# mfalxa/fakepta

Measured on AMD Instinct MI355X. Metric: residual samples/sec (TOA×realization) for 100-psr HD GWB; % FP64 peak, higher is better.
Workload: dtype f64

## Files before the change

fakepta_amd/_capi.py:

```python
import ctypes
import os
import threading

import numpy as np

_HERE = os.path.dirname(os.path.abspath(__file__))
_DEFAULT_LIB = os.path.join(_HERE, "lib", "libfakepta_amd.so")
LIB_PATH = os.environ.get("FAKEPTA_AMD_LIB", _DEFAULT_LIB)

if not os.path.exists(LIB_PATH):
    raise ImportError(
        f"fakepta_amd: HIP library not found at {LIB_PATH}. Build it with "
        "`python -c 'import __graft_entry__ as g; g.build()'` (or `make -C fakepta_amd/csrc`).")

_lib = ctypes.CDLL(LIB_PATH)

_c_int = ctypes.c_int
_i32, _i64, _u64 = ctypes.c_int32, ctypes.c_int64, ctypes.c_uint64
_dbl = ctypes.c_double
_vp = ctypes.c_void_p
_ctx_p = ctypes.c_void_p

_SIGS = [
    ("fpta_version", _c_int, []),
# ... 24 lines not shown
    ("fpta_batch_download", _c_int, [_ctx_p, _i32, _i32, _vp]),
    ("fpta_batch_device_out", _c_int, [_ctx_p, ctypes.POINTER(_vp), ctypes.POINTER(_i64), ctypes.POINTER(_i32)]),
    ("fpta_batch_checksums", _c_int, [_ctx_p, _vp]),
    ("fpta_batch_synth_checksums", _c_int, [_ctx_p, _u64, _i64, _i64, _i32, _vp]),
    ("fpta_batch_correlations", _c_int, [_ctx_p, _i32, _vp]),
    ("fpta_batch_info", _c_int, [_ctx_p, _vp]),
    ("fpta_batch_grid_info", _c_int, [_ctx_p, _vp]),
    ("fpta_batch_grid_info_n", _c_int, [_ctx_p, _vp, _i32]),
    ("fpta_set_option", _c_int, [_ctx_p, _i32, _i64]),
    ("fpta_kernel_stats", _c_int, [_ctx_p, _i32, ctypes.POINTER(_i64), ctypes.POINTER(_dbl)]),
    ("fpta_reset_stats", _c_int, [_ctx_p]),
    ("fpta_synchronize", _c_int, [_ctx_p]),
    ("fpta_debug_philox", _c_int, [_ctx_p, _i64, _vp, _vp, _vp]),
    ("fpta_debug_normals", _c_int, [_ctx_p, _i64, _vp, _vp]),
    ("fpta_debug_fill_out", _c_int, [_ctx_p, _dbl]),
    ("fpta_get_option", _c_int, [_ctx_p, _i32, ctypes.POINTER(_i64)]),
    ("fpta_build_flags", _c_int, []),
    ("fpta_batch_path_reason", ctypes.c_char_p, [_ctx_p]),
    ("fpta_multi_create", _c_int, [_i32, _vp, ctypes.POINTER(_vp)]),
    ("fpta_multi_destroy", _c_int, [_vp]),
    ("fpta_multi_last_error", ctypes.c_char_p, [_vp]),
    ("fpta_multi_size", _c_int, [_vp]),
    ("fpta_multi_context", _ctx_p, [_vp, _i32]),
    ("fpta_multi_set_toas", _c_int, [_vp, _i32, _vp, _vp, _vp]),
    ("fpta_multi_add_signal", _c_int, [_vp, _i32, _i32, _vp, _vp, _dbl, _dbl, _vp, _vp]),
    ("fpta_multi_set_white", _c_int, [_vp, _vp, _i64, _vp, _vp, _vp]),
    ("fpta_multi_set_option", _c_int, [_vp, _i32, _i64]),
    ("fpta_multi_synth", _c_int, [_vp, _u64, _i64, _i64, _i32, _vp]),
    ("fpta_multi_set_gather", _c_int, [_vp, _i32]),
    ("fpta_multi_last_gather", _c_int, [_vp]),
    ("fpta_comm_unique_id", _c_int, [_vp]),
    ("fpta_comm_init_rank", _c_int, [_ctx_p, _i32, _i32, _vp, ctypes.POINTER(_vp)]),
    ("fpta_comm_destroy", _c_int, [_vp]),
    ("fpta_comm_last_error", ctypes.c_char_p, [_vp]),
    ("fpta_comm_size", _c_int, [_vp, ctypes.POINTER(_i32), ctypes.POINTER(_i32)]),
    ("fpta_comm_max", _c_int, [_vp, ctypes.POINTER(_dbl)]),
    ("fpta_comm_gather", _c_int, [_vp, _vp, _i64, _vp]),
]
_OPTIONAL = {"fpta_debug_normals"}
for _name, _res, _args in _SIGS:
    try:
        _fn = getattr(_lib, _name)
    except AttributeError:
        if _name in _OPTIONAL and LIB_PATH != _DEFAULT_LIB:
            continue
        raise
    _fn.restype = _res
    _fn.argtypes = _args

EXPORTED = [s[0] for s in _SIGS]

OPT_SYNTH_PATH, OPT_MFMA_MIN_REAL, OPT_PROFILE, OPT_ANCHOR, OPT_VALU_VARIANT, OPT_FUSE_WHITE = 1, 2, 3, 4, 5, 6
OPT_GRID_WIDTH, OPT_GRID_SIGMA, OPT_GRID_MFMA, OPT_FUSE_CHECKSUMS = 7, 8, 9, 10
OPT_MIX_MFMA, OPT_OVERLAP, OPT_INTERP_LDS, OPT_GRID_COALESCE, OPT_INTERP_WS, OPT_SIDE_SPLIT = 11, 12, 13, 14, 15, 16
# ... 359 lines not shown
    def kernel_stats(self, which):
        n, ms = _i64(), _dbl()
        self._check(_lib.fpta_kernel_stats(self._h, int(which), ctypes.byref(n), ctypes.byref(ms)),
                    "fpta_kernel_stats")
        return n.value, ms.value

    def reset_stats(self):
        self._check(_lib.fpta_reset_stats(self._h), "fpta_reset_stats")

    def synchronize(self):
        self._check(_lib.fpta_synchronize(self._h), "fpta_synchronize")

    def debug_fill_out(self, value):
        self._check(_lib.fpta_debug_fill_out(self._h, float(value)), "fpta_debug_fill_out")

    def debug_philox(self, ctr, key):
        ctr = np.ascontiguousarray(ctr, dtype=np.uint32).reshape(-1, 4)
        key = np.ascontiguousarray(key, dtype=np.uint32)
        out = np.empty_like(ctr)
        self._check(_lib.fpta_debug_philox(self._h, len(ctr), _ptr(ctr), _ptr(key), _ptr(out)), "fpta_debug_philox")
        return out

    def debug_normals(self, words):
        words = np.ascontiguousarray(words, dtype=np.uint32).reshape(-1, 4)
        out = np.empty(words.shape, dtype=np.float64)
        self._check(_lib.fpta_debug_normals(self._h, len(words), _ptr(words), _ptr(out)), "fpta_debug_normals")
        return out


class _Borrowed(Context):
# ... 170 lines not shown
```

fakepta_amd/csrc/capi.hip:

```cpp
#include "capi_host.h"

namespace __attribute__((visibility("hidden"))) capi {

thread_local std::string g_err;


int fail(fpta_ctx* c, int code, const std::string& msg) {
  if (c) c->err = msg;
  g_err = msg;
  return code;
}

int hip_fail(fpta_ctx* c, hipError_t e, const char* what) {
  std::string m = std::string(what) + ": " + hipGetErrorString(e);
  return fail(c, e == hipErrorOutOfMemory ? FPTA_ENOMEM : FPTA_EDEVICE, m);
}

hipEvent_t get_event(fpta_ctx* c) {
  if (!c->pool.empty()) {
    hipEvent_t e = c->pool.back();
    c->pool.pop_back();
    return e;
  }
  hipEvent_t e = nullptr;
// ... 1531 lines not shown
int fpta_batch_grid_info(fpta_ctx* c, double* out) {
  const int rc = fpta_batch_grid_info_n(c, out, 9);
  return rc < 0 ? rc : FPTA_OK;
}

const char* fpta_batch_path_reason(const fpta_ctx* c) { return c ? c->path_reason.c_str() : ""; }

#ifdef FPTA_FUSED_PROF
extern "C" int fpta_debug_fused_prof(fpta_ctx* c, unsigned long long* host, int64_t n) {
  if (!c || !host || n <= 0 || !c->dbg_a.p || (size_t)n * 8 > c->dbg_a.cap) return FPTA_EINVAL;
  HIPCHK(c, hipMemcpy(host, c->dbg_a.p, (size_t)n * 8, hipMemcpyDeviceToHost), "profile download");
  return FPTA_OK;
}
#endif

int fpta_debug_fill_out(fpta_ctx* c, double value) {
  if (!c) return fail(nullptr, FPTA_EINVAL, "null ctx");
  if (!c->out_R) return fail(c, FPTA_ESTATE, "fill_out: nothing synthesized yet");
  HIPCHK(c, hipSetDevice(c->device), "hipSetDevice");
  const size_t n = (size_t)c->out_R * c->out_ld;
  std::vector<double> v(std::min<size_t>(n, (size_t)1 << 20), value);
  for (size_t i = 0; i < n; i += v.size())
    HIPCHK(c,
           hipMemcpyAsync(c->out.as<double>() + i, v.data(), sizeof(double) * std::min(v.size(), n - i),
                          hipMemcpyHostToDevice, c->stream),
           "fill_out copy");
  HIPCHK(c, hipStreamSynchronize(c->stream), "fill_out sync");
  return FPTA_OK;
}

// ... 30 lines not shown
```

fakepta_amd/csrc/capi_host.h:

```cpp
#pragma once
#include <hip/hip_runtime.h>
#include <rccl/rccl.h>

#include <algorithm>
#include <cmath>
#include <cstdio>
#include <cstdlib>
#include <cstring>
#include <string>
#include <vector>

#include "../../include/fakepta_amd.h"
#include "fpta_internal.h"

using namespace fpta;

namespace __attribute__((visibility("hidden"))) capi {

extern thread_local std::string g_err;

struct DevBuf {
  void* p = nullptr;
  size_t cap = 0;
  DevBuf() = default;
// ... 178 lines not shown
  DevBuf fused_q;
  bool fused_q_ready = false;
  int32_t out_R = 0;
  int64_t out_ld = 0;
  int synth_path = 0;
  int mfma_min_real = 16;
  int profile = 0;
  int anchor = 0;
  int valu_variant = 1;
  int fuse_white = 1;
  int fuse_sums = 0;
  int mix_mfma = 1;
  int overlap = 1;
  int interp_ws = 1;
  int last_interp = 0;
  double last_fma_interp = 0.0;
  int grid_coalesce = 1;
  int part_group = kPartGroup;
  int interp_psr = 1;
  int interp_wr = 0;
  int interp_fused = 1;
  DevBuf coef2;
  int coef_slot = 0;
  bool prev_psr = false;
  int fused_next_mix = 1;
  struct NextMix {
    bool valid = false;
    const Layout* layout = nullptr;
    uint64_t version = 0, seed = 0;
    int64_t real0 = 0;
// ... 138 lines not shown
```

fakepta_amd/csrc/fpta_internal.h:

```cpp
#pragma once
#include <hip/hip_runtime.h>
#include <stdint.h>

namespace fpta {

struct SegDesc {
  const double* w;
  const double* amp;
  const double* L;
  const double* LT;
  int32_t lt_ld, lt_rows;
  const uint8_t* mask;
  int64_t w_pstride;
  double idx;
  double freqf;
  int32_t nm;
  int32_t kind;
  int32_t col0;
  int32_t harmonic;
  int32_t l_lower;
  int32_t n_q;
};

struct SynthArgs {
// ... 186 lines not shown
  FusedHalf h;
  int32_t cu_pct;
  FusedMix mix;
};
#ifndef FPTA_FUSED_MIX_CU_PCT
#define FPTA_FUSED_MIX_CU_PCT 100
#endif
constexpr int kFusedQueueWords = 10;
constexpr int kFusedMixWord = 9;
#ifndef FPTA_FUSED_JOIN_SAFETY
#define FPTA_FUSED_JOIN_SAFETY 1.5
#endif
constexpr double kFusedJoinSafety = FPTA_FUSED_JOIN_SAFETY;
hipError_t launch_grid_fused(hipStream_t st, const SynthArgs& a, const GridBand& band, const FusedArgs& f,
                             int32_t nq_max, size_t lds_bytes, hipEvent_t ev0 = nullptr, hipEvent_t ev1 = nullptr,
                             bool half = false, int* kernel_out = nullptr);
constexpr int kFusedKernels = 9;
hipError_t launch_grid_interp_st(hipStream_t st, const SynthArgs& a, const GridBand& band, int32_t R_pad);
constexpr int kLdsGroup = 4, kLdsRowsMax = 144;
struct GridLds {
  const int4* groups;
  const int32_t* urows;
  const int32_t* lrows;
  int32_t n_groups, lds_rows;
};
hipError_t launch_grid_interp_lds(hipStream_t st, const SynthArgs& a, const GridBand& band, const GridLds& lds,
                                  int32_t R_pad);
constexpr int kUnionGroup = 4, kUnionRowsMax = 76, kUnionSigMax = 2, kUnionPitch = 130;
struct GridUnion {
  const int4* groups;
  const int32_t* urows;
// ... 68 lines not shown
```

fakepta_amd/csrc/fused_device.h:

```cpp
#pragma once
#include <hip/hip_runtime.h>

#include "grid_device.h"

namespace fpta {
#ifdef FPTA_FUSED_PROF
struct Prof {
  unsigned long long v[8] = {0, 0, 0, 0, 0, 0, 0, 0};
  unsigned long long t = 0;
  __device__ __forceinline__ void start() { t = clock64(); }
  __device__ __forceinline__ void lap(int i) {
    const unsigned long long n = clock64();
    v[i] += n - t;
    t = n;
  }
  __device__ __forceinline__ void count(int i) { ++v[i]; }
  __device__ __forceinline__ void flush(unsigned long long* out, int wave) {
    if (out && (threadIdx.x & 63) == 0)
      for (int i = 0; i < 8; ++i) out[((int64_t)blockIdx.x * 8 + wave) * 8 + i] = v[i];
  }
};
#else
struct Prof {
  __device__ __forceinline__ void start() {}
  __device__ __forceinline__ void lap(int) {}
  __device__ __forceinline__ void count(int) {}
  __device__ __forceinline__ void flush(unsigned long long*, int) {}
};
#endif

__device__ __forceinline__ double dpp_xor1(double x) {
  const int lo = __builtin_amdgcn_update_dpp(0, __double2loint(x), 0xB1, 0xF, 0xF, false);
  const int hi = __builtin_amdgcn_update_dpp(0, __double2hiint(x), 0xB1, 0xF, 0xF, false);
  return __hiloint2double(hi, lo);
}

__device__ __forceinline__ void fused_barrier() { asm volatile("s_barrier" ::: "memory"); }
__device__ __forceinline__ void fused_wait_lgkm0() { __builtin_amdgcn_s_waitcnt(15 | (3 << 14) | (7 << 4)); }

struct FusedQueue {
  int first, end;
  uint32_t* ticket;
  __device__ __forceinline__ FusedQueue(int n_items, uint32_t* q) {
    const int per = (n_items + 7) >> 3;
    const int x = blockIdx.x & 7;
    first = x * per;
    end = min(n_items, first + per);
    ticket = q + x;
  }
  __device__ __forceinline__ int fetch() const {
    const int t = (int)__hip_atomic_fetch_add(ticket, 1u, __ATOMIC_RELAXED, __HIP_MEMORY_SCOPE_AGENT);
    return first + t < end ? first + t : -1;
  }
// ... 4 lines not shown
```

fakepta_amd/csrc/grid_fused.hip:

```cpp
#include <hip/hip_runtime.h>
#include <hip/hip_ext.h>
#include <algorithm>
#include <atomic>
#include <type_traits>

#include "fused_device.h"

namespace fpta {

#ifndef FPTA_FUSED_DFT_PRIO
#define FPTA_FUSED_DFT_PRIO 3
#endif
#ifndef FPTA_HALF_STORE16
#define FPTA_HALF_STORE16 0
#endif
#ifndef FPTA_HALF_AHEAD
#define FPTA_HALF_AHEAD 2
#endif
constexpr int kFusedHalfAhead = FPTA_HALF_AHEAD;
#ifndef FPTA_HALF_PIN
#define FPTA_HALF_PIN 0
#endif

#ifndef FPTA_FUSED_CUT
// ... 86 lines not shown
  }
  const double am = ld_global(m.amp + k);
#pragma unroll
  for (int t = 0; t < NT; ++t)
#pragma unroll
    for (int h = 0; h < 2; ++h)
#pragma unroll
      for (int gg = 0; gg < 4; ++gg) {
        const int p = p0 + 16 * t + lg + 4 * gg;
        if (p < m.P) m.coef[((int64_t)p * m.K + m.col0 + 2 * k + h) * m.R_pad + r] = am * acc[t][h][gg];
      }
}

}

template <int NQ, bool ODD, bool GEN, bool HALF>
__global__ __launch_bounds__(64 * (kFusedIW + kFusedDW), 1) void k_grid_fused(SynthArgs a, GridBand band, FusedArgs f,
                                                                             int32_t n_rb, int32_t n_items) {
  static_assert(kFusedReal == 32 && kFusedPitch == 32 && kFusedGroupModes * kFusedReal / 2 == 64 * kFusedDW,
                "two realization tiles; one (mode, realization pair) of a 16-mode group per DFT lane");
  static_assert(!HALF || (NQ % 4 == 0 && kGridTT == 2 * kFusedHalfTT), "half bands: whole row groups, two halves");
  extern __shared__ __attribute__((aligned(16))) double lds[];
  const FusedQueue queue(n_items, f.queue);
  const int wave = __builtin_amdgcn_readfirstlane(threadIdx.x >> 6);
  const int lane = threadIdx.x & 63;
  const int lr = lane & 15, lg = lane >> 4;
  double* __restrict__ ring = lds + f.ring_off;
  uint32_t* sync = (uint32_t*)(ring + 2 * kFusedMaxSig * kFusedSlot);
  volatile int* qitem = (volatile int*)(sync + 4);
  if (threadIdx.x == 0) {
    *sync = 0u;
    ((volatile int*)sync)[8] = 0;
    ((volatile int*)sync)[9] = 0;
// ... 264 lines not shown
      t.nq = nq;
      interp_store_rows<2>(a, a.out, t, acc);
    }
    pf.lap(2);
  };
  auto process = [&](const Geo& g, const auto& cur, auto& pf, int ln) {
    if constexpr (HALF)
      process_half(g, cur, pf, ln);
    else
      process_full(g, cur, pf, ln);
  };

  if (wave >= kFusedIW) {
    const int dw = wave - kFusedIW;
    __builtin_amdgcn_s_setprio(FPTA_FUSED_DFT_PRIO);
    int js = -1, jrc = 0;
    {
      int j = dw;
#pragma unroll
      for (int s = 0; s < kFusedMaxSig; ++s) {
        if (s < f.n_sig && js < 0 && j < f.s[s].n_rc) {
          js = s;
          jrc = j;
        }
        if (s < f.n_sig) j -= f.s[s].n_rc;
      }
    }
    js = __builtin_amdgcn_readfirstlane(js);
    jrc = __builtin_amdgcn_readfirstlane(jrc);
    Prof pf;
    pf.start();
    uint32_t epoch = 0;
    auto dsync = [&]() {
      fused_wait_lgkm0();
      if (lane == 0) __hip_atomic_fetch_add(sync, 1u, __ATOMIC_RELAXED, __HIP_MEMORY_SCOPE_WORKGROUP);
      epoch += kFusedDW;
      while ((uint32_t)__builtin_amdgcn_readfirstlane(
                 (int)__hip_atomic_load(sync, __ATOMIC_RELAXED, __HIP_MEMORY_SCOPE_WORKGROUP)) < epoch)
        __builtin_amdgcn_s_sleep(1);
    };
    auto n_groups = [&](int nm) { return (((((nm + 1) >> 1) + 3) >> 2) + 1) >> 1; };
    int ng[kFusedMaxSig];
    int n_it = 0;
#pragma unroll
    for (int s = 0; s < kFusedMaxSig; ++s) {
      ng[s] = s < f.n_sig ? n_groups(f.s[s].nm) : 0;
      n_it = max(n_it, ng[s]);
    }
    const FusedSig& jf = f.s[js < 0 ? 0 : js];
    const int64_t jts = (int64_t)jf.ntq * jf.ldq, jld4 = 4 * (int64_t)jf.ldq;
    auto jtq_now = [&]() {
      const int ln = lane_now();
      return jf.tq + (int64_t)(ln >> 4) * jf.ldq + 32 * jrc + 2 * (ln & 15);
    };
    const int jnq0 = (((jf.nm + 1) >> 1) + 3) >> 2, jnq1 = ((jf.nm >> 1) + 3) >> 2;
    const int jng = js < 0 ? 0 : (jnq0 + 1) >> 1;
    d4 C[2][2][2], S[2][2][2];
    struct DrawIn {
      dbl2 x0[kFusedTerms], x1[kFusedTerms];
    };
    auto draw_load = [&](const FusedSig& fs, int g, int p, int r0, DrawIn& in) {
      const int didx = dw * 64 + lane_now(), dmm = didx >> 4, drl = 2 * (didx & 15);
      const int m = kFusedGroupModes * g + dmm, r = r0 + drl;
#pragma unroll
      for (int i = 0; i < kFusedTerms; ++i) {
        const bool on = i < fs.n_terms;
        const int nmi = on ? fs.term_nm[i] : 2;
        const int mi = min(m, nmi - 1);
        const double* src0;
        int64_t step;
        if (on && fs.term_kind[i] == 1) {
          src0 = a.coef + ((int64_t)p * a.K + fs.term_col0[i] + 2 * mi) * a.R_pad + r;
          step = a.R_pad;
        } else {
          src0 = (on ? fs.term_amp[i] : a.coef) + (int64_t)p * nmi + (mi & ~1);
          step = 0;
        }
        in.x0[i] = ld_global((const dbl2*)src0);
        in.x1[i] = ld_global((const dbl2*)(src0 + step));
      }
    };
    auto draw_finish = [&](const FusedSig& fs, int g, int p, int r0, double* __restrict__ slot_s, const DrawIn& in) {
      const int didx = dw * 64 + lane_now(), dmm = didx >> 4, drl = 2 * (didx & 15);
      const int m = kFusedGroupModes * g + dmm, r = r0 + drl;
      const uint64_t gr = (uint64_t)(f.real0 + r);
      double bc[2] = {0.0, 0.0}, bs[2] = {0.0, 0.0};
      bool first = true;
      auto add = [&](bool use, const double (&pc)[2], const double (&ps)[2]) {
#pragma unroll
        for (int h = 0; h < 2; ++h) {
          bc[h] = use ? (first ? pc[h] : bc[h] + pc[h]) : bc[h];
          bs[h] = use ? (first ? ps[h] : bs[h] + ps[h]) : bs[h];
        }
        first = first && !use;
      };
      const bool ok0 = r < a.n_real, ok1 = r + 1 < a.n_real;
      auto normals = [&](int seg, double (&z)[4]) {
        if (!ODD) {
          gp_pair2((uint32_t)m, (uint32_t)p, (uint32_t)seg, gr, f.k0, f.k1, z);
        } else {
          gp_normal2((uint32_t)m, (uint32_t)p, (uint32_t)seg, gr, f.k0, f.k1, z[0], z[1]);
          gp_normal2((uint32_t)m, (uint32_t)p, (uint32_t)seg, gr + 1, f.k0, f.k1, z[2], z[3]);
        }
        z[0] = ok0 ? z[0] : 0.0;
        z[1] = ok0 ? z[1] : 0.0;
        z[2] = ok1 ? z[2] : 0.0;
        z[3] = ok1 ? z[3] : 0.0;
      };
#pragma unroll
      for (int i = 0; i < kFusedTerms; ++i) {
        if (i >= fs.n_terms) continue;
        double pc[2], ps[2];
        if (GEN && fs.term_kind[i] == 0) {
          double z[4];
          normals(fs.term_seg[i], z);
          const double amp = (m & 1) ? in.x0[i].y : in.x0[i].x;
          pc[0] = opaque(amp * z[0]);
          ps[0] = opaque(amp * z[1]);
          pc[1] = opaque(amp * z[2]);
          ps[1] = opaque(amp * z[3]);
        } else {
          pc[0] = in.x0[i].x;
          pc[1] = in.x0[i].y;
          ps[0] = in.x1[i].x;
          ps[1] = in.x1[i].y;
        }
        add(m < fs.nm && m < fs.term_nm[i], pc, ps);
      }
      for (int i = kFusedTerms; i < fs.n_terms; ++i) {
        const int mi = min(m, fs.term_nm[i] - 1);
        double pc[2], ps[2];
        if (GEN && fs.term_kind[i] == 0) {
          double z[4];
          normals(fs.term_seg[i], z);
          const double amp = ld_global(fs.term_amp[i] + (int64_t)p * fs.term_nm[i] + mi);
          pc[0] = opaque(amp * z[0]);
          ps[0] = opaque(amp * z[1]);
          pc[1] = opaque(amp * z[2]);
          ps[1] = opaque(amp * z[3]);
        } else {
          const double* cp = a.coef + ((int64_t)p * a.K + fs.term_col0[i] + 2 * mi) * a.R_pad + r;
          const dbl2 vc = ld_global((const dbl2*)cp), vs = ld_global((const dbl2*)(cp + a.R_pad));
          pc[0] = vc.x;
          pc[1] = vc.y;
// ... 46 lines not shown
    int sb = 0;
    auto build = [&](int k) {
      const int item = item_of(k);
      const int p = item / n_rb, r0 = (item - p * n_rb) * kFusedReal;
      const int item1n = item_of(k + 1);
      const bool nx = item1n >= 0;
      const int item1 = nx ? item1n : item;
      const int p1 = item1 / n_rb, r1 = (item1 - p1 * n_rb) * kFusedReal;
#pragma unroll
      for (int par = 0; par < 2; ++par)
#pragma unroll
        for (int h = 0; h < 2; ++h)
#pragma unroll
          for (int t = 0; t < 2; ++t) C[par][h][t] = S[par][h][t] = d4{0.0, 0.0, 0.0, 0.0};
      if (k == 0) {
#pragma unroll
        for (int s = 0; s < kFusedMaxSig; ++s) {
          if (s >= f.n_sig) continue;
          DrawIn in;
          draw_load(f.s[s], 0, p, r0, in);
          draw_finish(f.s[s], 0, p, r0, slot_of(sb, s), in);
        }
        pf.lap(6);
        dsync();
        pf.lap(2);
      }
      for (int g = 0; g < n_it; ++g) {
        const bool last = g + 1 == n_it;
        const int dp = last ? p1 : p, dr = last ? r1 : r0;
        Tabs tb;
        tables(g, tb);
        DrawIn in[kFusedMaxSig];
#pragma unroll
        for (int s = 0; s < kFusedMaxSig; ++s)
          draw_load(f.s[s], last ? 0 : min(g + 1, max(ng[s], 1) - 1), dp, dr, in[s]);
        pf.lap(0);
        if (g < jng) steps(sb + g, g, tb);
        pf.lap(1);
#pragma unroll
        for (int s = 0; s < kFusedMaxSig; ++s)
          if (last ? nx && s < f.n_sig : g + 1 < ng[s])
            draw_finish(f.s[s], last ? 0 : g + 1, dp, dr, slot_of(sb + g + 1, s), in[s]);
        pf.lap(6);
        dsync();
        pf.lap(2);
        pf.count(5);
      }
      sb = (sb + n_it) & 1;
    };
    auto write_grid = [&]() {
      if (js >= 0) {
        const int j0 = 32 * jrc;
        const int nf = jf.nf, Q = nf >> 2, H = nf >> 1;
        double* __restrict__ gcol = lds + (int64_t)jf.lrow0 * kFusedPitch + lr;
#pragma unroll
        for (int h = 0; h < 2; ++h)
#pragma unroll
          for (int gg = 0; gg < 4; ++gg) {
// ... 121 lines not shown
    g1 = geo(k + 1);
    ex0 = ex1;
    ex1 = false;
    if (kc < 0) {
      const int cc = next(kc);
      load(cc >= 0 ? cc : g0.c0, o0, lane);
    }
  }
  pf.flush(f.prof, wave);
  }
  mix_tiles();
  fused_barrier();
  if (wave < kFusedIW) finish();
}

hipError_t launch_grid_fused(hipStream_t st, const SynthArgs& a, const GridBand& band, const FusedArgs& f,
                             int32_t nq_max, size_t lds_bytes, hipEvent_t ev0, hipEvent_t ev1, bool half,
                             int* kernel_out) {
  if (band.n_chunks <= 0 || band.vmax < 4 || f.join_reserve < 0 || band.vmax % 4 != 0 || a.R_pad % kFusedReal != 0 || a.w_on ||
      a.accumulate || a.part || !f.lrows || !f.psr_c0 || f.n_sig <= 0 || f.n_sig > kFusedMaxSig ||
      lds_bytes > (size_t)kFusedLdsMax || nq_max <= 0 || f.ring_off < 0 || f.fq < kFusedNQ || f.fq % 4 != 0 ||
      !f.queue || (size_t)(f.ring_off + 2 * kFusedMaxSig * kFusedSlot) * sizeof(double) + 48 > lds_bytes)
    return hipErrorInvalidValue;
  if (half && (!f.h.chunks || !f.h.lrows || !f.h.wd || f.h.fq < kFusedHalfNQ || f.h.fq % 4 != 0 || f.h.vmax < 8 ||
               f.h.vmax % 8 != 0))
    return hipErrorInvalidValue;
  int jobs = 0;
  for (int s = 0; s < f.n_sig; ++s) {
    const FusedSig& fs = f.s[s];
    const int nq = ((((fs.nm + 1) >> 1) + 3) >> 2);
    if (fs.nf % 4 != 0 || !fs.tq || fs.n_rc != (fs.nf / 4 + 32) / 32 || fs.ldq < 32 * fs.n_rc || 4 * nq > fs.ntq ||
        fs.n_terms <= 0 || fs.n_terms > kDftGenTerms || fs.lrow0 < 0 || (fs.lrow0 + fs.nf) * kFusedPitch > f.ring_off)
      return hipErrorInvalidValue;
    for (int i = 0; i < fs.n_terms; ++i)
      if (fs.term_nm[i] <= 0 || fs.term_nm[i] > fs.nm || (fs.term_kind[i] == 0 && (!fs.term_amp[i] || fs.term_nm[i] % 2)) ||
          (fs.term_kind[i] == 1 && (!a.coef || fs.term_col0[i] < 0 || fs.term_col0[i] + 2 * fs.term_nm[i] > a.K)))
        return hipErrorInvalidValue;
    jobs += fs.n_rc;
  }
  if (jobs > kFusedDW) return hipErrorInvalidValue;
  const FusedMix& m = f.mix;
  if (m.n_tiles != 0 &&
      (m.n_tiles < 0 || !m.LT || !m.amp || !m.coef || m.P <= 0 || m.P > kFusedMixMaxP || m.lt_ld < 16 * ((m.P + 15) / 16) ||
       m.lt_rows < 4 * ((m.P + 3) / 4) || m.n_q <= 0 || m.n_q > m.P || m.nm <= 0 || m.R_pad <= 0 ||
       m.R_pad % 16 != 0 || m.n_real <= 0 || m.n_real > m.R_pad || (int64_t)m.n_tiles != (int64_t)m.nm * (m.R_pad / 16) * ((m.P + kFusedMixGroup - 1) / kFusedMixGroup) ||
       m.col0 < 0 || m.col0 + 2 * m.nm > m.K || m.real0 < 0 || m.real0 + m.n_real > ((int64_t)1 << 32)))
    return hipErrorInvalidValue;
  const int32_t n_rb = a.R_pad / kFusedReal;
  const int64_t items = (int64_t)a.P * n_rb;
  if (items > 0x7FFFFFFF || items <= 0) return hipErrorInvalidValue;
  int dev = 0;
  if (hipGetDevice(&dev) != hipSuccess || dev < 0 || dev >= 64) return hipErrorInvalidDevice;
  static std::atomic<int> n_cus[64];
  static std::atomic<bool> attr_set[64][kFusedKernels];
  int n_cu = n_cus[dev].load(std::memory_order_relaxed);
  if (n_cu <= 0) {
    if (hipDeviceGetAttribute(&n_cu, hipDeviceAttributeMultiprocessorCount, dev) != hipSuccess || n_cu <= 0) n_cu = 256;
    n_cus[dev].store(n_cu, std::memory_order_relaxed);
  }
  const int64_t cus = f.cu_pct > 0 && f.cu_pct < 100 ? std::max<int64_t>(8, (int64_t)n_cu * f.cu_pct / 100) : n_cu;
  const int64_t grid = std::min<int64_t>((items + 7) / 8 * 8, (cus + 7) / 8 * 8);
  bool gen = false;
  for (int s = 0; s < f.n_sig; ++s)
    for (int i = 0; i < f.s[s].n_terms; ++i) gen = gen || f.s[s].term_kind[i] == 0;
  const bool odd = gen && (f.real0 & 1);
  const int ki = half ? 6 + (gen ? 1 + odd : 0) : (nq_max <= 8 ? 0 : 3) + (gen ? 1 + odd : 0);
  using K = void (*)(SynthArgs, GridBand, FusedArgs, int32_t, int32_t);
  static const K kernels[kFusedKernels] = {
      k_grid_fused<8, false, false, false>,  k_grid_fused<8, false, true, false>,  k_grid_fused<8, true, true, false>,
      k_grid_fused<12, false, false, false>, k_grid_fused<12, false, true, false>, k_grid_fused<12, true, true, false>,
      k_grid_fused<kFusedHalfNQ, false, false, true>, k_grid_fused<kFusedHalfNQ, false, true, true>,
      k_grid_fused<kFusedHalfNQ, true, true, true>};
  const K kernel = kernels[ki];
  if (!attr_set[dev][ki].load(std::memory_order_acquire)) {
    hipError_t e = hipFuncSetAttribute((const void*)kernel, hipFuncAttributeMaxDynamicSharedMemorySize, kFusedLdsMax);
    if (e != hipSuccess) return e;
    attr_set[dev][ki].store(true, std::memory_order_release);
  }
  FusedArgs fa = f;
  for (int s = f.n_sig; s < kFusedMaxSig; ++s) fa.s[s] = f.s[0];
  (void)hipGetLastError();
  int32_t n_rb_arg = n_rb, items_arg = (int32_t)items;
  void* args[] = {(void*)&a, (void*)&band, (void*)&fa, (void*)&n_rb_arg, (void*)&items_arg};
  const hipError_t e = hipExtLaunchKernel((const void*)kernel, dim3((unsigned)grid),
                                          dim3(64 * (kFusedIW + kFusedDW)), args, lds_bytes, st, ev0, ev1, 0);
  if (e == hipSuccess && kernel_out) *kernel_out = ki;
  return e;
}

}
```

fakepta_amd/csrc/grid_host.hip:

```cpp
#include "capi_host.h"

namespace __attribute__((visibility("hidden"))) capi {

void gauss_legendre(int n, std::vector<double>& x, std::vector<double>& wt) {
  x.assign(n, 0.0);
  wt.assign(n, 0.0);
  for (int i = 0; i < (n + 1) / 2; ++i) {
    double z = std::cos(M_PI * (i + 0.75) / (n + 0.5)), dp = 1.0;
    for (int it = 0; it < 100; ++it) {
      double p0 = 1.0, p1 = z;
      for (int k = 2; k <= n; ++k) {
        const double p2 = ((2.0 * k - 1.0) * z * p1 - (k - 1.0) * p0) / k;
        p0 = p1;
        p1 = p2;
      }
      dp = n * (z * p1 - p0) / (z * z - 1.0);
      const double dz = p1 / dp;
      z -= dz;
      if (std::fabs(dz) < 1e-16) break;
    }
    x[i] = -z;
    x[n - 1 - i] = z;
    wt[i] = wt[n - 1 - i] = 2.0 / ((1.0 - z * z) * dp * dp);
  }
// ... 872 lines not shown
          fs.term_amp[fs.n_terms] = sd2.amp;
          ++fs.n_terms;
        }
      } else {
        fs.term_kind[0] = 1;
        fs.term_seg[0] = G.anchor[s];
        fs.term_nm[0] = d.nm;
        fs.term_col0[0] = d.col0;
        fs.n_terms = 1;
      }
    }
    {
      int it_max = 0, gen = 0;
      for (int32_t s = 0; s < f.n_sig; ++s) {
        const int nm = f.s[s].nm;
        it_max = std::max(it_max, (((((nm + 1) >> 1) + 3) >> 2) + 1) >> 1);
        for (int i = 0; i < f.s[s].n_terms; ++i) gen += f.s[s].term_kind[i] == 0;
      }
      const double build = it_max * (32.0 + 20.0 * gen);
      const double chunk = G.mean_v + 12.0;
      f.join_reserve = (int32_t)std::min(1.0e6, std::ceil(kFusedJoinSafety * kFusedIW * build / chunk));
    }
    f.ring_off = (G.fused_lrow0.back() + G.segs.back()->nf) * kFusedPitch;
    {
      bool sep_mix = false;
      for (const Seg* sg : L.segs) sep_mix = sep_mix || (sg->d.kind == 1 && L.P > kGenMixMaxP);
      f.cu_pct = pipe && sep_mix ? FPTA_FUSED_MIX_CU_PCT : 100;
    }
    f.lrows = G.frows.as<int32_t>();
    f.fq = G.fused_fq;
    f.psr_c0 = G.psr_c0.as<int32_t>();
// ... 35 lines not shown
      m.lt_ld = d.lt_ld;
      m.lt_rows = d.lt_rows;
      m.P = L.P;
      m.K = a.K;
      m.col0 = d.col0;
      m.R_pad = R_pad;
      m.n_real = a.n_real;
      m.n_q = d.n_q;
      m.lower = d.l_lower;
      m.seg = nms;
      m.nm = d.nm;
      m.n_tiles = d.nm * (R_pad / 16) * ((L.P + kFusedMixGroup - 1) / kFusedMixGroup);
    }
    hipEvent_t e0 = kt.start_ev();
    int ki = 0;
    HIPCHK(c, kt.checked(launch_grid_fused(c->stream, a, band, f, nq, G.fused_lds, e0, kt.stop_ev(), half, &ki)),
           "k_grid_fused launch");
    kind = kInterpKindFused0 + ki;
    if (f.mix.n_tiles > 0) {
      fpta_ctx::NextMix& nx = c->next_mix;
      nx.valid = true;
      nx.layout = &L;
      nx.version = L.version;
      nx.seed = blk_seed;
      nx.real0 = f.mix.real0;
      nx.n_real = a.n_real;
      nx.R_pad = R_pad;
      nx.seg = nms;
      nx.buf = c->coef2.p;
      nx.done = nullptr;
      c->next_mix_made = true;
// ... 12 lines not shown
    kind = 1;
    HIPCHK(c, launch_grid_interp_ws(c->stream, a, band, R_pad), "k_grid_interp_ws launch");
#ifdef FPTA_DIAG_KERNELS
  } else if (c->interp_lds && G.lds_ok && !a.w_on) {
    kind = 3;
    band.pgfirst = nullptr;
    band.n_pg = G.n_chunks;
    GridLds lds{G.groups.as<int4>(), G.urows.as<int32_t>(), G.lrows.as<int32_t>(), G.n_groups, G.lds_rows};
    HIPCHK(c, launch_grid_interp_lds(c->stream, a, band, lds, R_pad), "k_grid_interp_lds launch");
#endif
  } else {
    kind = 0;
    HIPCHK(c, launch_grid_interp_mfma(c->stream, a, band, R_pad), "k_grid_interp_mfma launch");
  }
  c->last_interp = 1 + kind * 4 + (a.w_on ? 2 : 0) + (a.part ? 1 : 0);
  if (kind < kInterpKindFused0) c->last_fma_interp = G.fma_interp;
  if (pipe) {
    HIPCHK(c, hipEventRecord(c->ev_gfree[gi], c->stream), "event record");
    if (c->next_mix_made) c->next_mix.done = c->ev_gfree[gi];
    c->gfree_set[gi] = true;
    c->gbuf = gi ^ 1;
  }
  if (a.part) {
    c->part_ready = true;
    c->part_chunks = band.n_pg;
    c->part_rpad = R_pad;
  }
  return FPTA_OK;
}

// ... 2 lines not shown
```

include/fakepta_amd.h:

```cpp
#ifndef FAKEPTA_AMD_H
#define FAKEPTA_AMD_H

#include <stdint.h>

#ifdef __cplusplus
extern "C" {
#endif

#define FPTA_OK 0
#define FPTA_EINVAL (-22)
#define FPTA_ENOMEM (-12)
#define FPTA_EDEVICE (-19)
#define FPTA_ESTATE (-77)

typedef struct fpta_ctx fpta_ctx;

#define FPTA_VERSION 10300
int fpta_version(void);
int fpta_create(int device, fpta_ctx** out);
int fpta_destroy(fpta_ctx* ctx);
const char* fpta_last_error(const fpta_ctx* ctx);
int fpta_device_count(int* n);


// ... 147 lines not shown
#define FPTA_K_SYNTH 2
#define FPTA_K_WHITE 3
#define FPTA_K_DENSE 4
#define FPTA_K_GRID 5
#define FPTA_K_CW 6
#define FPTA_K_EPHEM 7
#define FPTA_K_N 8
int fpta_kernel_stats(fpta_ctx* ctx, int32_t which, int64_t* count, double* total_ms);
int fpta_reset_stats(fpta_ctx* ctx);
int fpta_synchronize(fpta_ctx* ctx);

int fpta_debug_philox(fpta_ctx* ctx, int64_t n, const uint32_t* ctr, const uint32_t* key,
                      uint32_t* out);
int fpta_debug_normals(fpta_ctx* ctx, int64_t n, const uint32_t* words, double* out);
int fpta_debug_fill_out(fpta_ctx* ctx, double value);

#ifdef __cplusplus
}
#endif
#endif
```

Before: 384.0 billion.

## Specialize fused grid kernel for common signal-term shapes at compile time

Adds compile-time shape variants of the fused grid/DFT kernel for the two common signal configurations (gen+load pair, or a single load). In these variants the per-term branching is resolved statically, unnecessary loads and table builds are skipped, and a vm-count wait is placed before the sync. The original generic kernel is kept as a fallback, selected on the host by matching the shape. This targets the runtime branching and wasted loads in the DFT waves, at the cost of doubling the number of kernel instantiations and adding a new explicit memory wait.

```diff
diff --git a/fakepta_amd/_capi.py b/fakepta_amd/_capi.py
--- a/fakepta_amd/_capi.py
+++ b/fakepta_amd/_capi.py
@@ -62,6 +62,7 @@
     ("fpta_debug_philox", _c_int, [_ctx_p, _i64, _vp, _vp, _vp]),
     ("fpta_debug_normals", _c_int, [_ctx_p, _i64, _vp, _vp]),
     ("fpta_debug_fill_out", _c_int, [_ctx_p, _dbl]),
+    ("fpta_debug_fused_shape", _c_int, [_ctx_p, _vp]),
     ("fpta_get_option", _c_int, [_ctx_p, _i32, ctypes.POINTER(_i64)]),
     ("fpta_build_flags", _c_int, []),
     ("fpta_batch_path_reason", ctypes.c_char_p, [_ctx_p]),
@@ -85,7 +86,7 @@
     ("fpta_comm_max", _c_int, [_vp, ctypes.POINTER(_dbl)]),
     ("fpta_comm_gather", _c_int, [_vp, _vp, _i64, _vp]),
 ]
-_OPTIONAL = {"fpta_debug_normals"}
+_OPTIONAL = {"fpta_debug_normals", "fpta_debug_fused_shape"}
 for _name, _res, _args in _SIGS:
     try:
         _fn = getattr(_lib, _name)
@@ -475,6 +476,11 @@
     def debug_fill_out(self, value):
         self._check(_lib.fpta_debug_fill_out(self._h, float(value)), "fpta_debug_fill_out")
 
+    def debug_fused_shape(self):
+        shape = np.zeros(1, dtype=np.int32)
+        self._check(_lib.fpta_debug_fused_shape(self._h, _ptr(shape)), "fpta_debug_fused_shape")
+        return int(shape[0])
+
     def debug_philox(self, ctr, key):
         ctr = np.ascontiguousarray(ctr, dtype=np.uint32).reshape(-1, 4)
         key = np.ascontiguousarray(key, dtype=np.uint32)
diff --git a/fakepta_amd/csrc/capi.hip b/fakepta_amd/csrc/capi.hip
--- a/fakepta_amd/csrc/capi.hip
+++ b/fakepta_amd/csrc/capi.hip
@@ -1569,6 +1569,12 @@
 }
 #endif
 
+int fpta_debug_fused_shape(fpta_ctx* c, int32_t* shape) {
+  if (!c || !shape) return fail(c, FPTA_EINVAL, "debug_fused_shape: bad arguments");
+  *shape = c->last_interp > 0 ? c->last_fused_shape : -1;
+  return FPTA_OK;
+}
+
 int fpta_debug_fill_out(fpta_ctx* c, double value) {
   if (!c) return fail(nullptr, FPTA_EINVAL, "null ctx");
   if (!c->out_R) return fail(c, FPTA_ESTATE, "fill_out: nothing synthesized yet");
diff --git a/fakepta_amd/csrc/capi_host.h b/fakepta_amd/csrc/capi_host.h
--- a/fakepta_amd/csrc/capi_host.h
+++ b/fakepta_amd/csrc/capi_host.h
@@ -216,6 +216,7 @@
   int overlap = 1;
   int interp_ws = 1;
   int last_interp = 0;
+  int last_fused_shape = -1;
   double last_fma_interp = 0.0;
   int grid_coalesce = 1;
   int part_group = kPartGroup;
diff --git a/fakepta_amd/csrc/fpta_internal.h b/fakepta_amd/csrc/fpta_internal.h
--- a/fakepta_amd/csrc/fpta_internal.h
+++ b/fakepta_amd/csrc/fpta_internal.h
@@ -1,6 +1,8 @@
 #pragma once
 #include <hip/hip_runtime.h>
 #include <stdint.h>
+
+#include "fused_sched.h"
 
 namespace fpta {
 
@@ -224,7 +226,7 @@
 constexpr double kFusedJoinSafety = FPTA_FUSED_JOIN_SAFETY;
 hipError_t launch_grid_fused(hipStream_t st, const SynthArgs& a, const GridBand& band, const FusedArgs& f,
                              int32_t nq_max, size_t lds_bytes, hipEvent_t ev0 = nullptr, hipEvent_t ev1 = nullptr,
-                             bool half = false, int* kernel_out = nullptr);
+                             bool half = false, int* kernel_out = nullptr, int* shape_out = nullptr);
 constexpr int kFusedKernels = 9;
 hipError_t launch_grid_interp_st(hipStream_t st, const SynthArgs& a, const GridBand& band, int32_t R_pad);
 constexpr int kLdsGroup = 4, kLdsRowsMax = 144;
diff --git a/fakepta_amd/csrc/fused_device.h b/fakepta_amd/csrc/fused_device.h
--- a/fakepta_amd/csrc/fused_device.h
+++ b/fakepta_amd/csrc/fused_device.h
@@ -37,6 +37,7 @@
 
 __device__ __forceinline__ void fused_barrier() { asm volatile("s_barrier" ::: "memory"); }
 __device__ __forceinline__ void fused_wait_lgkm0() { __builtin_amdgcn_s_waitcnt(15 | (3 << 14) | (7 << 4)); }
+__device__ __forceinline__ void fused_wait_vm0() { __builtin_amdgcn_s_waitcnt((7 << 4) | (15 << 8)); }
 
 struct FusedQueue {
   int first, end;
diff --git a/fakepta_amd/csrc/fused_sched.h b/fakepta_amd/csrc/fused_sched.h
--- /dev/null
+++ b/fakepta_amd/csrc/fused_sched.h
@@ -0,0 +1,43 @@
+#pragma once
+#include <cstdint>
+
+#if defined(__HIPCC__)
+#define FPTA_SCHED_HD __host__ __device__
+#else
+#define FPTA_SCHED_HD
+#endif
+
+namespace fpta {
+
+constexpr int kFusedShapeAny = 0;
+constexpr int kFusedShapeGenLoad = 1;
+constexpr int kFusedShapeLoad = 2;
+constexpr int kFusedSlotAny = -1, kFusedSlotNone = 0, kFusedSlotGen = 1, kFusedSlotLoad = 2;
+FPTA_SCHED_HD constexpr int fused_shape_nsig(int shape) {
+  return shape == kFusedShapeGenLoad ? 2 : shape == kFusedShapeLoad ? 1 : 0;
+}
+FPTA_SCHED_HD constexpr int fused_shape_slot(int shape, int s, int i) {
+  return shape == kFusedShapeAny       ? kFusedSlotAny
+         : shape == kFusedShapeGenLoad ? (i == 0 ? kFusedSlotGen : (s == 0 && i == 1 ? kFusedSlotLoad : kFusedSlotNone))
+                                       : (s == 0 && i == 0 ? kFusedSlotLoad : kFusedSlotNone);
+}
+
+FPTA_SCHED_HD constexpr int fused_shape_match(int n_sig, const int32_t* n_terms, const int32_t (*kind)[2]) {
+  return n_sig == 2 && n_terms[0] == 2 && kind[0][0] == 0 && kind[0][1] == 1 && n_terms[1] == 1 && kind[1][0] == 0
+             ? kFusedShapeGenLoad
+         : n_sig == 1 && n_terms[0] == 1 && kind[0][0] == 1 ? kFusedShapeLoad
+                                                            : kFusedShapeAny;
+}
+
+FPTA_SCHED_HD constexpr int32_t fused_ksteps(int32_t nm, int par) { return (((nm + (par ? 0 : 1)) >> 1) + 3) >> 2; }
+FPTA_SCHED_HD constexpr int32_t fused_groups(int32_t nm) { return (fused_ksteps(nm, 0) + 1) >> 1; }
+
+FPTA_SCHED_HD constexpr int32_t fused_iterations(int32_t ng0, int32_t ng1) { return ng0 > ng1 ? ng0 : ng1; }
+FPTA_SCHED_HD constexpr bool fused_steps(int32_t jng, int32_t g) { return g < jng; }
+FPTA_SCHED_HD constexpr bool fused_draw_loads(int32_t ng_s, int32_t g, bool last) { return last || g + 1 < ng_s; }
+FPTA_SCHED_HD constexpr bool fused_draws(int32_t ng_s, int32_t g, bool last, bool nx) { return last ? nx : g + 1 < ng_s; }
+FPTA_SCHED_HD constexpr int32_t fused_draw_group(int32_t g, bool last) { return last ? 0 : g + 1; }
+
+}
+
+#undef FPTA_SCHED_HD
diff --git a/fakepta_amd/csrc/grid_fused.hip b/fakepta_amd/csrc/grid_fused.hip
--- a/fakepta_amd/csrc/grid_fused.hip
+++ b/fakepta_amd/csrc/grid_fused.hip
@@ -124,9 +124,11 @@
 
 }
 
-template <int NQ, bool ODD, bool GEN, bool HALF>
-__global__ __launch_bounds__(64 * (kFusedIW + kFusedDW), 1) void k_grid_fused(SynthArgs a, GridBand band, FusedArgs f,
-                                                                             int32_t n_rb, int32_t n_items) {
+template <int NQ, bool ODD, bool GEN, bool HALF, int SHAPE>
+__device__ __forceinline__ void grid_fused_body(const SynthArgs& a, const GridBand& band, const FusedArgs& f,
+                                                int32_t n_rb, int32_t n_items) {
+  static_assert(kFusedTerms == 2 && kFusedMaxSig == 2, "fused_shape_slot's slots and signals (c0, c1)");
+  static_assert(SHAPE == kFusedShapeAny || GEN == (SHAPE == kFusedShapeGenLoad), "a shape fixes whether terms are drawn");
   static_assert(kFusedReal == 32 && kFusedPitch == 32 && kFusedGroupModes * kFusedReal / 2 == 64 * kFusedDW,
                 "two realization tiles; one (mode, realization pair) of a 16-mode group per DFT lane");
   static_assert(!HALF || (NQ % 4 == 0 && kGridTT == 2 * kFusedHalfTT), "half bands: whole row groups, two halves");
@@ -421,16 +423,18 @@
   if (wave >= kFusedIW) {
     const int dw = wave - kFusedIW;
     __builtin_amdgcn_s_setprio(FPTA_FUSED_DFT_PRIO);
+    constexpr int kNSig = fused_shape_nsig(SHAPE);
+    const int n_sig = kNSig ? kNSig : f.n_sig;
     int js = -1, jrc = 0;
     {
       int j = dw;
 #pragma unroll
       for (int s = 0; s < kFusedMaxSig; ++s) {
-        if (s < f.n_sig && js < 0 && j < f.s[s].n_rc) {
+        if (s < n_sig && js < 0 && j < f.s[s].n_rc) {
           js = s;
           jrc = j;
         }
-        if (s < f.n_sig) j -= f.s[s].n_rc;
+        if (s < n_sig) j -= f.s[s].n_rc;
       }
     }
     js = __builtin_amdgcn_readfirstlane(js);
@@ -446,48 +450,62 @@
                  (int)__hip_atomic_load(sync, __ATOMIC_RELAXED, __HIP_MEMORY_SCOPE_WORKGROUP)) < epoch)
         __builtin_amdgcn_s_sleep(1);
     };
-    auto n_groups = [&](int nm) { return (((((nm + 1) >> 1) + 3) >> 2) + 1) >> 1; };
     int ng[kFusedMaxSig];
-    int n_it = 0;
-#pragma unroll
-    for (int s = 0; s < kFusedMaxSig; ++s) {
-      ng[s] = s < f.n_sig ? n_groups(f.s[s].nm) : 0;
-      n_it = max(n_it, ng[s]);
-    }
+#pragma unroll
+    for (int s = 0; s < kFusedMaxSig; ++s) ng[s] = s < n_sig ? fused_groups(f.s[s].nm) : 0;
+    const int n_it = fused_iterations(ng[0], ng[1]);
     const FusedSig& jf = f.s[js < 0 ? 0 : js];
     const int64_t jts = (int64_t)jf.ntq * jf.ldq, jld4 = 4 * (int64_t)jf.ldq;
     auto jtq_now = [&]() {
       const int ln = lane_now();
       return jf.tq + (int64_t)(ln >> 4) * jf.ldq + 32 * jrc + 2 * (ln & 15);
     };
-    const int jnq0 = (((jf.nm + 1) >> 1) + 3) >> 2, jnq1 = ((jf.nm >> 1) + 3) >> 2;
-    const int jng = js < 0 ? 0 : (jnq0 + 1) >> 1;
+    const int jnq0 = fused_ksteps(jf.nm, 0), jnq1 = fused_ksteps(jf.nm, 1);
+    const int jng = js < 0 ? 0 : fused_groups(jf.nm);
     d4 C[2][2][2], S[2][2][2];
     struct DrawIn {
       dbl2 x0[kFusedTerms], x1[kFusedTerms];
     };
-    auto draw_load = [&](const FusedSig& fs, int g, int p, int r0, DrawIn& in) {
+    std::integral_constant<int, 0> c0;
+    std::integral_constant<int, 1> c1;
+    auto draw_load = [&](auto sc, int g, int p, int r0, DrawIn& in) {
+      constexpr int s = decltype(sc)::value;
+      const FusedSig& fs = f.s[s];
       const int didx = dw * 64 + lane_now(), dmm = didx >> 4, drl = 2 * (didx & 15);
       const int m = kFusedGroupModes * g + dmm, r = r0 + drl;
-#pragma unroll
-      for (int i = 0; i < kFusedTerms; ++i) {
-        const bool on = i < fs.n_terms;
-        const int nmi = on ? fs.term_nm[i] : 2;
-        const int mi = min(m, nmi - 1);
-        const double* src0;
-        int64_t step;
-        if (on && fs.term_kind[i] == 1) {
-          src0 = a.coef + ((int64_t)p * a.K + fs.term_col0[i] + 2 * mi) * a.R_pad + r;
-          step = a.R_pad;
-        } else {
-          src0 = (on ? fs.term_amp[i] : a.coef) + (int64_t)p * nmi + (mi & ~1);
-          step = 0;
-        }
-        in.x0[i] = ld_global((const dbl2*)src0);
-        in.x1[i] = ld_global((const dbl2*)(src0 + step));
-      }
-    };
-    auto draw_finish = [&](const FusedSig& fs, int g, int p, int r0, double* __restrict__ slot_s, const DrawIn& in) {
+      auto slot = [&](auto ic) {
+        constexpr int i = decltype(ic)::value, kind = fused_shape_slot(SHAPE, s, i);
+        if constexpr (kind == kFusedSlotGen) {
+          const int nmi = fs.term_nm[i], mi = min(m, nmi - 1);
+          in.x0[i] = ld_global((const dbl2*)(fs.term_amp[i] + (int64_t)p * nmi + (mi & ~1)));
+        } else if constexpr (kind == kFusedSlotLoad) {
+          const int mi = min(m, fs.term_nm[i] - 1);
+          const double* src0 = a.coef + ((int64_t)p * a.K + fs.term_col0[i] + 2 * mi) * a.R_pad + r;
+          in.x0[i] = ld_global((const dbl2*)src0);
+          in.x1[i] = ld_global((const dbl2*)(src0 + a.R_pad));
+        } else if constexpr (kind == kFusedSlotAny) {
+          const bool on = i < fs.n_terms;
+          const int nmi = on ? fs.term_nm[i] : 2;
+          const int mi = min(m, nmi - 1);
+          const double* src0;
+          int64_t step;
+          if (on && fs.term_kind[i] == 1) {
+            src0 = a.coef + ((int64_t)p * a.K + fs.term_col0[i] + 2 * mi) * a.R_pad + r;
+            step = a.R_pad;
+          } else {
+            src0 = (on ? fs.term_amp[i] : a.coef) + (int64_t)p * nmi + (mi & ~1);
+            step = 0;
+          }
+          in.x0[i] = ld_global((const dbl2*)src0);
+          in.x1[i] = ld_global((const dbl2*)(src0 + step));
+        }
+      };
+      slot(c0);
+      slot(c1);
+    };
+    auto draw_finish = [&](auto sc, int g, int p, int r0, double* __restrict__ slot_s, const DrawIn& in) {
+      constexpr int s = decltype(sc)::value;
+      const FusedSig& fs = f.s[s];
       const int didx = dw * 64 + lane_now(), dmm = didx >> 4, drl = 2 * (didx & 15);
       const int m = kFusedGroupModes * g + dmm, r = r0 + drl;
       const uint64_t gr = (uint64_t)(f.real0 + r);
@@ -503,22 +521,24 @@
       };
       const bool ok0 = r < a.n_real, ok1 = r + 1 < a.n_real;
       auto normals = [&](int seg, double (&z)[4]) {
+        uint32_t k0 = f.k0, k1 = f.k1;
+        if (SHAPE != kFusedShapeAny) asm volatile("" : "+s"(k0), "+s"(k1));
         if (!ODD) {
-          gp_pair2((uint32_t)m, (uint32_t)p, (uint32_t)seg, gr, f.k0, f.k1, z);
+          gp_pair2((uint32_t)m, (uint32_t)p, (uint32_t)seg, gr, k0, k1, z);
         } else {
-          gp_normal2((uint32_t)m, (uint32_t)p, (uint32_t)seg, gr, f.k0, f.k1, z[0], z[1]);
-          gp_normal2((uint32_t)m, (uint32_t)p, (uint32_t)seg, gr + 1, f.k0, f.k1, z[2], z[3]);
+          gp_normal2((uint32_t)m, (uint32_t)p, (uint32_t)seg, gr, k0, k1, z[0], z[1]);
+          gp_normal2((uint32_t)m, (uint32_t)p, (uint32_t)seg, gr + 1, k0, k1, z[2], z[3]);
         }
         z[0] = ok0 ? z[0] : 0.0;
         z[1] = ok0 ? z[1] : 0.0;
         z[2] = ok1 ? z[2] : 0.0;
         z[3] = ok1 ? z[3] : 0.0;
       };
-#pragma unroll
-      for (int i = 0; i < kFusedTerms; ++i) {
-        if (i >= fs.n_terms) continue;
+      auto term = [&](auto ic) {
+        constexpr int i = decltype(ic)::value, kind = fused_shape_slot(SHAPE, s, i);
+        if (kind == kFusedSlotNone || (kind == kFusedSlotAny && i >= fs.n_terms)) return;
         double pc[2], ps[2];
-        if (GEN && fs.term_kind[i] == 0) {
+        if (kind == kFusedSlotGen || (kind == kFusedSlotAny && GEN && fs.term_kind[i] == 0)) {
           double z[4];
           normals(fs.term_seg[i], z);
           const double amp = (m & 1) ? in.x0[i].y : in.x0[i].x;
@@ -533,8 +553,10 @@
           ps[1] = in.x1[i].y;
         }
         add(m < fs.nm && m < fs.term_nm[i], pc, ps);
-      }
-      for (int i = kFusedTerms; i < fs.n_terms; ++i) {
+      };
+      term(c0);
+      term(c1);
+      for (int i = kFusedTerms; SHAPE == kFusedShapeAny && i < fs.n_terms; ++i) {
         const int mi = min(m, fs.term_nm[i] - 1);
         double pc[2], ps[2];
         if (GEN && fs.term_kind[i] == 0) {
@@ -611,34 +633,46 @@
 #pragma unroll
           for (int t = 0; t < 2; ++t) C[par][h][t] = S[par][h][t] = d4{0.0, 0.0, 0.0, 0.0};
       if (k == 0) {
-#pragma unroll
-        for (int s = 0; s < kFusedMaxSig; ++s) {
-          if (s >= f.n_sig) continue;
+        auto first = [&](auto sc) {
+          constexpr int s = decltype(sc)::value;
+          if (s >= n_sig) return;
           DrawIn in;
-          draw_load(f.s[s], 0, p, r0, in);
-          draw_finish(f.s[s], 0, p, r0, slot_of(sb, s), in);
-        }
+          draw_load(sc, 0, p, r0, in);
+          draw_finish(sc, 0, p, r0, slot_of(sb, s), in);
+        };
+        first(c0);
+        first(c1);
         pf.lap(6);
         dsync();
         pf.lap(2);
       }
+      constexpr bool kAny = SHAPE == kFusedShapeAny;
       for (int g = 0; g < n_it; ++g) {
         const bool last = g + 1 == n_it;
         const int dp = last ? p1 : p, dr = last ? r1 : r0;
         Tabs tb;
-        tables(g, tb);
+        if (kAny) tables(g, tb);
         DrawIn in[kFusedMaxSig];
-#pragma unroll
-        for (int s = 0; s < kFusedMaxSig; ++s)
-          draw_load(f.s[s], last ? 0 : min(g + 1, max(ng[s], 1) - 1), dp, dr, in[s]);
+        auto load = [&](auto sc) {
+          constexpr int s = decltype(sc)::value;
+          if (kAny || (s < kNSig && fused_draw_loads(ng[s], g, last)))
+            draw_load(sc, last ? 0 : min(g + 1, max(ng[s], 1) - 1), dp, dr, in[s]);
+        };
+        load(c0);
+        load(c1);
+        if (!kAny && fused_steps(jng, g)) tables(g, tb);
         pf.lap(0);
-        if (g < jng) steps(sb + g, g, tb);
+        if (fused_steps(jng, g)) steps(sb + g, g, tb);
         pf.lap(1);
-#pragma unroll
-        for (int s = 0; s < kFusedMaxSig; ++s)
-          if (last ? nx && s < f.n_sig : g + 1 < ng[s])
-            draw_finish(f.s[s], last ? 0 : g + 1, dp, dr, slot_of(sb + g + 1, s), in[s]);
+        auto finish_draw = [&](auto sc) {
+          constexpr int s = decltype(sc)::value;
+          if (s < n_sig && fused_draws(ng[s], g, last, nx))
+            draw_finish(sc, fused_draw_group(g, last), dp, dr, slot_of(sb + g + 1, s), in[s]);
+        };
+        finish_draw(c0);
+        finish_draw(c1);
         pf.lap(6);
+        if (!kAny) fused_wait_vm0();
         dsync();
         pf.lap(2);
         pf.count(5);
@@ -790,9 +824,34 @@
   if (wave < kFusedIW) finish();
 }
 
+template <int NQ, bool ODD, bool GEN, bool HALF>
+__global__ __launch_bounds__(64 * (kFusedIW + kFusedDW), 1) void k_grid_fused(SynthArgs a, GridBand band, FusedArgs f,
+                                                                             int32_t n_rb, int32_t n_items) {
+  grid_fused_body<NQ, ODD, GEN, HALF, GEN ? kFusedShapeGenLoad : kFusedShapeLoad>(a, band, f, n_rb, n_items);
+}
+template <int NQ, bool ODD, bool GEN, bool HALF>
+__global__ __launch_bounds__(64 * (kFusedIW + kFusedDW), 1) void k_grid_fused_any(SynthArgs a, GridBand band,
+                                                                                 FusedArgs f, int32_t n_rb,
+                                                                                 int32_t n_items) {
+  grid_fused_body<NQ, ODD, GEN, HALF, kFusedShapeAny>(a, band, f, n_rb, n_items);
+}
+
+#ifndef FPTA_FUSED_SHAPES
+#define FPTA_FUSED_SHAPES 1
+#endif
+static int fused_shape_of(const FusedArgs& f) {
+  int32_t n_terms[kFusedMaxSig], kind[kFusedMaxSig][2];
+  for (int s = 0; s < kFusedMaxSig; ++s) {
+    n_terms[s] = f.s[s].n_terms;
+    kind[s][0] = f.s[s].term_kind[0];
+    kind[s][1] = f.s[s].term_kind[1];
+  }
+  return FPTA_FUSED_SHAPES ? fused_shape_match(f.n_sig, n_terms, kind) : kFusedShapeAny;
+}
+
 hipError_t launch_grid_fused(hipStream_t st, const SynthArgs& a, const GridBand& band, const FusedArgs& f,
                              int32_t nq_max, size_t lds_bytes, hipEvent_t ev0, hipEvent_t ev1, bool half,
-                             int* kernel_out) {
+                             int* kernel_out, int* shape_out) {
   if (band.n_chunks <= 0 || band.vmax < 4 || f.join_reserve < 0 || band.vmax % 4 != 0 || a.R_pad % kFusedReal != 0 || a.w_on ||
       a.accumulate || a.part || !f.lrows || !f.psr_c0 || f.n_sig <= 0 || f.n_sig > kFusedMaxSig ||
       lds_bytes > (size_t)kFusedLdsMax || nq_max <= 0 || f.ring_off < 0 || f.fq < kFusedNQ || f.fq % 4 != 0 ||
@@ -804,7 +863,7 @@
   int jobs = 0;
   for (int s = 0; s < f.n_sig; ++s) {
     const FusedSig& fs = f.s[s];
-    const int nq = ((((fs.nm + 1) >> 1) + 3) >> 2);
+    const int nq = fused_ksteps(fs.nm, 0);
     if (fs.nf % 4 != 0 || !fs.tq || fs.n_rc != (fs.nf / 4 + 32) / 32 || fs.ldq < 32 * fs.n_rc || 4 * nq > fs.ntq ||
         fs.n_terms <= 0 || fs.n_terms > kDftGenTerms || fs.lrow0 < 0 || (fs.lrow0 + fs.nf) * kFusedPitch > f.ring_off)
       return hipErrorInvalidValue;
@@ -828,7 +887,7 @@
   int dev = 0;
   if (hipGetDevice(&dev) != hipSuccess || dev < 0 || dev >= 64) return hipErrorInvalidDevice;
   static std::atomic<int> n_cus[64];
-  static std::atomic<bool> attr_set[64][kFusedKernels];
+  static std::atomic<bool> attr_set[64][2][kFusedKernels];
   int n_cu = n_cus[dev].load(std::memory_order_relaxed);
   if (n_cu <= 0) {
     if (hipDeviceGetAttribute(&n_cu, hipDeviceAttributeMultiprocessorCount, dev) != hipSuccess || n_cu <= 0) n_cu = 256;
@@ -842,16 +901,22 @@
   const bool odd = gen && (f.real0 & 1);
   const int ki = half ? 6 + (gen ? 1 + odd : 0) : (nq_max <= 8 ? 0 : 3) + (gen ? 1 + odd : 0);
   using K = void (*)(SynthArgs, GridBand, FusedArgs, int32_t, int32_t);
-  static const K kernels[kFusedKernels] = {
-      k_grid_fused<8, false, false, false>,  k_grid_fused<8, false, true, false>,  k_grid_fused<8, true, true, false>,
-      k_grid_fused<12, false, false, false>, k_grid_fused<12, false, true, false>, k_grid_fused<12, true, true, false>,
-      k_grid_fused<kFusedHalfNQ, false, false, true>, k_grid_fused<kFusedHalfNQ, false, true, true>,
-      k_grid_fused<kFusedHalfNQ, true, true, true>};
-  const K kernel = kernels[ki];
-  if (!attr_set[dev][ki].load(std::memory_order_acquire)) {
+  static const K kernels[2][kFusedKernels] = {
+      {k_grid_fused_any<8, false, false, false>, k_grid_fused_any<8, false, true, false>,
+       k_grid_fused_any<8, true, true, false>, k_grid_fused_any<12, false, false, false>,
+       k_grid_fused_any<12, false, true, false>, k_grid_fused_any<12, true, true, false>,
+       k_grid_fused_any<kFusedHalfNQ, false, false, true>, k_grid_fused_any<kFusedHalfNQ, false, true, true>,
+       k_grid_fused_any<kFusedHalfNQ, true, true, true>},
+      {k_grid_fused<8, false, false, false>, k_grid_fused<8, false, true, false>, k_grid_fused<8, true, true, false>,
+       k_grid_fused<12, false, false, false>, k_grid_fused<12, false, true, false>, k_grid_fused<12, true, true, false>,
+       k_grid_fused<kFusedHalfNQ, false, false, true>, k_grid_fused<kFusedHalfNQ, false, true, true>,
+       k_grid_fused<kFusedHalfNQ, true, true, true>}};
+  const int shaped = fused_shape_of(f) == (gen ? kFusedShapeGenLoad : kFusedShapeLoad) ? 1 : 0;
+  const K kernel = kernels[shaped][ki];
+  if (!attr_set[dev][shaped][ki].load(std::memory_order_acquire)) {
     hipError_t e = hipFuncSetAttribute((const void*)kernel, hipFuncAttributeMaxDynamicSharedMemorySize, kFusedLdsMax);
     if (e != hipSuccess) return e;
-    attr_set[dev][ki].store(true, std::memory_order_release);
+    attr_set[dev][shaped][ki].store(true, std::memory_order_release);
   }
   FusedArgs fa = f;
   for (int s = f.n_sig; s < kFusedMaxSig; ++s) fa.s[s] = f.s[0];
@@ -861,6 +926,7 @@
   const hipError_t e = hipExtLaunchKernel((const void*)kernel, dim3((unsigned)grid),
                                           dim3(64 * (kFusedIW + kFusedDW)), args, lds_bytes, st, ev0, ev1, 0);
   if (e == hipSuccess && kernel_out) *kernel_out = ki;
+  if (e == hipSuccess && shape_out) *shape_out = shaped ? (gen ? kFusedShapeGenLoad : kFusedShapeLoad) : kFusedShapeAny;
   return e;
 }
 
diff --git a/fakepta_amd/csrc/grid_host.hip b/fakepta_amd/csrc/grid_host.hip
--- a/fakepta_amd/csrc/grid_host.hip
+++ b/fakepta_amd/csrc/grid_host.hip
@@ -910,7 +910,7 @@
       int it_max = 0, gen = 0;
       for (int32_t s = 0; s < f.n_sig; ++s) {
         const int nm = f.s[s].nm;
-        it_max = std::max(it_max, (((((nm + 1) >> 1) + 3) >> 2) + 1) >> 1);
+        it_max = std::max(it_max, fused_groups(nm));
         for (int i = 0; i < f.s[s].n_terms; ++i) gen += f.s[s].term_kind[i] == 0;
       }
       const double build = it_max * (32.0 + 20.0 * gen);
@@ -976,7 +976,8 @@
     }
     hipEvent_t e0 = kt.start_ev();
     int ki = 0;
-    HIPCHK(c, kt.checked(launch_grid_fused(c->stream, a, band, f, nq, G.fused_lds, e0, kt.stop_ev(), half, &ki)),
+    HIPCHK(c, kt.checked(launch_grid_fused(c->stream, a, band, f, nq, G.fused_lds, e0, kt.stop_ev(), half, &ki,
+                                           &c->last_fused_shape)),
            "k_grid_fused launch");
     kind = kInterpKindFused0 + ki;
     if (f.mix.n_tiles > 0) {
@@ -1019,6 +1020,7 @@
     HIPCHK(c, launch_grid_interp_mfma(c->stream, a, band, R_pad), "k_grid_interp_mfma launch");
   }
   c->last_interp = 1 + kind * 4 + (a.w_on ? 2 : 0) + (a.part ? 1 : 0);
+  if (kind < kInterpKindFused0) c->last_fused_shape = -1;
   if (kind < kInterpKindFused0) c->last_fma_interp = G.fma_interp;
   if (pipe) {
     HIPCHK(c, hipEventRecord(c->ev_gfree[gi], c->stream), "event record");
diff --git a/include/fakepta_amd.h b/include/fakepta_amd.h
--- a/include/fakepta_amd.h
+++ b/include/fakepta_amd.h
@@ -185,6 +185,7 @@
                       uint32_t* out);
 int fpta_debug_normals(fpta_ctx* ctx, int64_t n, const uint32_t* words, double* out);
 int fpta_debug_fill_out(fpta_ctx* ctx, double value);
+int fpta_debug_fused_shape(fpta_ctx* ctx, int32_t* shape);
 
 #ifdef __cplusplus
 }
```

Result: faster. 395.9 billion (median of 6 runs) (+3.1%).
